# marella/ctransformers

Measured on NVIDIA H100. Metric: decode tokens/s Llama-2-7B Q4_K_M b=1, higher is better.
Workload: dtype int8 (q4_K/q6_K weights x q8_K activations, mma.sync u8 x s8 -> exact int32), fp32 combine in the reference's order

## Files before the change

ctransformers_b200/csrc/engine.cu:

```cuda
#include "engine.cuh"

#include <algorithm>
#include <chrono>
#include <cstdio>
#include <cstring>
#include <stdexcept>

#include "attention.cuh"
#include "matvec.cuh"
#include "prefill.cuh"
#include "repack.cuh"
#include "sample_gpu.cuh"
#include "stream.cuh"
#include "tables.hpp"
#include "tp_nccl.hpp"

namespace ctb {

#define CTB_CUDA(expr)                                                                                         \
  do {                                                                                                         \
    cudaError_t e__ = (expr);                                                                                  \
    if (e__ != cudaSuccess)                                                                                    \
      throw std::runtime_error(std::string("CUDA error: ") + cudaGetErrorString(e__) + " at " + __FILE__ + ":" + \
                               std::to_string(__LINE__) + " (" #expr ")" + watchdog_note());                   \
// ... 775 lines not shown
  if (launches) *launches = (long)sel.size();
  stream_ = user; launches_per_step_ = keep;
  cudaStreamDestroy(cap);
  cudaEvent_t e0, e1;
  CTB_CUDA(cudaEventCreate(&e0)); CTB_CUDA(cudaEventCreate(&e1));
  for (int i = 0; i < 3; i++) CTB_CUDA(cudaGraphLaunch(ex, stream_));
  CTB_CUDA(cudaEventRecord(e0, stream_));
  for (int i = 0; i < reps; i++) CTB_CUDA(cudaGraphLaunch(ex, stream_));
  CTB_CUDA(cudaEventRecord(e1, stream_));
  CTB_CUDA(cudaStreamSynchronize(stream_));
  float ms = 0;
  cudaEventElapsedTime(&ms, e0, e1);
  cudaEventDestroy(e0); cudaEventDestroy(e1); cudaGraphExecDestroy(ex);
  return (double)ms / reps;
}

long Engine::trace_step(int token, int n_past, unsigned long long* out, long cap_words) {
  DeviceGuard dev_guard(device_);
  if (tp_.world > 1) throw std::runtime_error("not available in tensor-parallel mode (every rank must run the same launches)");
  spec_pending_ = false; spec_deferred_ = false; spec_pos_ = -1; spec_streak_ = 0;
  const int n = n_body_ + 1;
  for (int i = 0; i < n; i++)
    if (ops_[i].ph.kind == PH_MATVEC && !ops_[i].stream) return 0;
  const long need = 2L * n + 8L * n * step_grid_;
  if (need > cap_words) return -need;
  unsigned long long* buf = nullptr;
  CTB_CUDA(cudaMalloc(&buf, (size_t)n * step_grid_ * 64));
  CTB_CUDA(cudaMemset(buf, 0, (size_t)n * step_grid_ * 64));
  StepLaunch L;
  L.grid = step_grid_; L.n_slots = step_slots_; L.smem = step_smem_; L.gen = !attn_fast_hd(hp_.head_dim());
  if (h_state_cap_ < 1) { h_state_cap_ = 512; CTB_CUDA(cudaMallocHost(&h_state_, (size_t)h_state_cap_ * 16)); }
  for (int rep = 0; rep < 3; rep++) {
    h_state_[0] = token; h_state_[1] = n_past; h_state_[2] = 0; h_state_[3] = n_past + 1;
    CTB_CUDA(cudaMemcpyAsync(d_state_, h_state_, 16, cudaMemcpyHostToDevice, stream_));
    CTB_CUDA(launch_step(L, stream_, d_prog_, d_bounds_, n, d_sync_, false, buf));
    CTB_CUDA(cudaStreamSynchronize(stream_));
  }
  for (int i = 0; i < n; i++) { out[2 * i] = (unsigned long long)ops_[i].ph.kind; out[2 * i + 1] = (unsigned long long)ops_[i].mvk; }
  const cudaError_t e = cudaMemcpy(out + 2 * n, buf, (size_t)n * step_grid_ * 64, cudaMemcpyDeviceToHost);
  cudaFree(buf);
  CTB_CUDA(e);
  return n;
}

void Engine::destroy_graphs() {
  if (graph_full_) cudaGraphExecDestroy(graph_full_);
  if (graph_nolog_) cudaGraphExecDestroy(graph_nolog_);
  if (graph_greedy_) cudaGraphExecDestroy(graph_greedy_);
  graph_full_ = graph_nolog_ = graph_greedy_ = nullptr;
}

void Engine::build_graphs() {
  destroy_graphs();
  if (!d_tokens_out_) {
    tokens_out_cap_ = std::max(hp_.n_ctx, 4096);
    CTB_CUDA(cudaMalloc(&d_tokens_out_, (size_t)tokens_out_cap_ * 4));
    CTB_CUDA(cudaMallocHost(&h_tokens_out_, (size_t)tokens_out_cap_ * 4));
  }
  cudaStream_t user = stream_;
  cudaStream_t cap;
  CTB_CUDA(cudaStreamCreateWithFlags(&cap, cudaStreamNonBlocking));
  stream_ = cap;
// ... 309 lines not shown
```

ctransformers_b200/csrc/matvec.cuh:

```cuda
#pragma once
#include "device_types.cuh"
#include "attention.cuh"

namespace ctb {

#ifndef CTB_THREADS
#define CTB_THREADS 512
#endif
constexpr int MV_THREADS = CTB_THREADS;
constexpr int MV_WARPS = MV_THREADS / 32;
constexpr int MV_ROWS = 4;
constexpr int MV_MAX_SEG = 3;

enum : int { NORM_NONE = 0, NORM_RMS = 1, NORM_LAYER = 2 };
enum : int { EPI_STORE = 0, EPI_ADD = 1, EPI_GELU = 2, EPI_ADD2 = 3, EPI_SILU = 4 };

#ifndef ST_WATCHDOG_NS
#define ST_WATCHDOG_NS 4000000000ull
#endif
#ifndef XC_WATCHDOG_NS
#define XC_WATCHDOG_NS 30000000000ull
#endif
enum WaitCode : int {
  W_GRID_BARRIER = 1, W_FOLD_FLAG, W_FREE_WEIGHT_SLOT, W_WEIGHT_ITEM, W_FREE_K_SLOT, W_FREE_V_SLOT, W_K_ITEM, W_V_ITEM, W_XCHG,
// ... 73 lines not shown
  return a;
}

__device__ __forceinline__ int q8k_word_offset(int b, int s, int l) { return ((b * 2 + (s >> 2)) * 8 + l) * 16 + (s & 3) * 4; }


template <bool CG = false>
__device__ __forceinline__ void load16(const float* p, int valid, float (&v)[16]) {
  if (valid >= 16) {
    float4 a, b, c, d;
    if (CG) { a = __ldcg((const float4*)p); b = __ldcg((const float4*)p + 1); c = __ldcg((const float4*)p + 2); d = __ldcg((const float4*)p + 3); }
    else { a = __ldg((const float4*)p); b = __ldg((const float4*)p + 1); c = __ldg((const float4*)p + 2); d = __ldg((const float4*)p + 3); }
    v[0] = a.x; v[1] = a.y; v[2] = a.z; v[3] = a.w; v[4] = b.x; v[5] = b.y; v[6] = b.z; v[7] = b.w;
    v[8] = c.x; v[9] = c.y; v[10] = c.z; v[11] = c.w; v[12] = d.x; v[13] = d.y; v[14] = d.z; v[15] = d.w;
  } else {
#pragma unroll
    for (int e = 0; e < 16; e++) v[e] = e < valid ? (CG ? __ldcg(p + e) : __ldg(p + e)) : 0.f;
  }
}

template <int NT, int BAR>
__device__ __forceinline__ double block_sum_f64(double s, double* red ) {
  s = warp_sum(s);
  bar_sync<BAR, NT>();
  if ((threadIdx.x & 31) == 0) red[threadIdx.x >> 5] = s;
  bar_sync<BAR, NT>();
  double t = 0.0;
#pragma unroll
  for (int w = 0; w < NT / 32; w++) t += red[w];
  return t;
}
template <int NT, int BAR>
__device__ __forceinline__ void block_sum2_max_f64(double& s, double& a, double& g, double* red) {
  constexpr int NW = NT / 32;
#pragma unroll
  for (int o = 16; o > 0; o >>= 1) {
    s += __shfl_xor_sync(0xffffffffu, s, o);
    a += __shfl_xor_sync(0xffffffffu, a, o);
    g = fmax(g, __shfl_xor_sync(0xffffffffu, g, o));
  }
  bar_sync<BAR, NT>();
  if ((threadIdx.x & 31) == 0) { red[threadIdx.x >> 5] = s; red[NW + (threadIdx.x >> 5)] = a; red[2 * NW + (threadIdx.x >> 5)] = g; }
  bar_sync<BAR, NT>();
  s = 0.0;
  a = 0.0;
#pragma unroll
  for (int w = 0; w < NW; w++) { s += red[w]; a += red[NW + w]; g = fmax(g, red[2 * NW + w]); }
}

__device__ __forceinline__ uint32_t pack4(const int* q) {
  return (uint32_t)(q[0] & 0xff) | ((uint32_t)(q[1] & 0xff) << 8) | ((uint32_t)(q[2] & 0xff) << 16) | ((uint32_t)(q[3] & 0xff) << 24);
}

__device__ __forceinline__ void load16_ll(const uint2* p, unsigned epoch, float (&u)[16]) {
  uint4 q[8];
  bounded_wait([&] {
    bool ok = true;
#pragma unroll
    for (int j = 0; j < 8; j++) {
      asm volatile("ld.volatile.global.v4.u32 {%0,%1,%2,%3}, [%4];" : "=r"(q[j].x), "=r"(q[j].y), "=r"(q[j].z), "=r"(q[j].w) : "l"(p + 2 * j) : "memory");
    }
#pragma unroll
    for (int j = 0; j < 8; j++) ok &= q[j].y == epoch && q[j].w == epoch;
    return ok;
// ... 52 lines not shown
  double seq = 0.0;
  for (int base = 0; base < K; base += 512) {
    float v[16];
    load16x<XC>(xs, base + lane * 16, K - base - lane * 16, v, epoch);
    for (int l = 0; l < 32; l++)
#pragma unroll
      for (int i = 0; i < 16; i++) {
        float t = __shfl_sync(0xffffffffu, v[i], l);
        if (kind == NORM_TERM_DEV) t = __fsub_rn(t, mean);
        if (base + l * 16 + i < K) seq += kind == NORM_TERM_X ? (double)t : (double)__fmul_rn(t, t);
      }
  }
  return seq;
}

template <int NT, int BAR, bool XC>
__device__ __forceinline__ float norm_stat(double s, double a, double g, bool a_is_s, int kind, float mean, const MVParams& xs, double* red,
                                           unsigned epoch) {
  const int K = xs.K;
  if (a_is_s) a = s = block_sum_f64<NT, BAR>(s, red);
  else block_sum2_max_f64<NT, BAR>(s, a, g, red);
  if (!isfinite(s) || (!a_is_s && __dmul_ru(a, g) < 0x1p52)) return (float)(s / (double)K);
  const double e = __dmul_ru(a, (double)K * 0x1.0000001p-52);
  const float lo = (float)(__dsub_rd(s, e) / (double)K), hi = (float)(__dadd_ru(s, e) / (double)K);
  if (lo == hi) return lo;
  const double seq = threadIdx.x < 32 ? seq_sum_warp0<XC>(xs.x, xs.x2, xs.x_mode, xs.x_parts, xs.x_stride, K, kind, mean, epoch) : 0.0;
  bar_sync<BAR, NT>();
  if (threadIdx.x == 0) red[0] = seq;
  bar_sync<BAR, NT>();
  return (float)(red[0] / (double)K);
}

template <int NT, int BAR, bool XC = false>
__device__ __forceinline__ void stage_activation(const MVParams& xs, const NormPre& np, int act, uint8_t* smem, double* red, bool write_norm, unsigned epoch = 0) {
  const float* nw = xs.norm_w;
  const float* nb_ = xs.norm_b;
  float* norm_out = xs.norm_out;
  const int norm_mode = xs.norm_mode, K = xs.K;
  const float eps = xs.eps;
  const int t = threadIdx.x, lane = t & 31;
  const int passes = (K + NT * 16 - 1) / (NT * 16);
  float mean = 0.f, scale = 1.f;
  float v0[16];
  load16x<XC>(xs, t * 16, K - t * 16, v0, epoch);
  if (norm_mode == NORM_RMS) {
    double ss = 0.0;
    for (int ps = 0; ps < passes; ps++) {
      const int base = (ps * NT + t) * 16;
      if ((base & ~511) >= K) continue;
      float v[16];
      if (ps == 0) {
#pragma unroll
        for (int e = 0; e < 16; e++) v[e] = v0[e];
      } else load16x<XC>(xs, base, K - base, v, epoch);
#pragma unroll
      for (int e = 0; e < 16; e++) ss += (double)__fmul_rn(v[e], v[e]);
    }
    const float m = norm_stat<NT, BAR, XC>(ss, ss, 0.0, true, NORM_TERM_SQ, 0.f, xs, red, epoch);
    scale = __fdiv_rn(1.0f, __fsqrt_rn(__fadd_rn(m, eps)));
  } else if (norm_mode == NORM_LAYER) {
    double s1 = 0.0, a1 = 0.0;
    unsigned emin = 255;
    for (int ps = 0; ps < passes; ps++) {
      const int base = (ps * NT + t) * 16;
      if ((base & ~511) >= K) continue;
      float v[16];
      load16x<XC>(xs, base, K - base, v, epoch);
#pragma unroll
      for (int e = 0; e < 16; e++) {
        s1 += (double)v[e];
        a1 += (double)fabsf(v[e]);
        emin = min_exp(emin, v[e]);
      }
    }
    mean = norm_stat<NT, BAR, XC>(s1, a1, lsb_inv(emin), false, NORM_TERM_X, 0.f, xs, red, epoch);
    double s2 = 0.0;
    for (int ps = 0; ps < passes; ps++) {
      const int base = (ps * NT + t) * 16;
      if ((base & ~511) >= K) continue;
      float v[16];
      load16x<XC>(xs, base, K - base, v, epoch);
#pragma unroll
      for (int e = 0; e < 16; e++) { const float d = (base + e < K) ? __fsub_rn(v[e], mean) : 0.f; s2 += (double)__fmul_rn(d, d); }
    }
    const float var = norm_stat<NT, BAR, XC>(s2, s2, 0.0, true, NORM_TERM_DEV, mean, xs, red, epoch);
    scale = __fdiv_rn(1.0f, __fsqrt_rn(__fadd_rn(var, eps)));
  }
  int8_t* qs = (int8_t*)smem;
  const size_t off = ((size_t)K + 15) & ~(size_t)15;
  float* dd = (float*)(smem + off);
  int16_t* bs = (int16_t*)(smem + off + q8k_d_bytes(K));
  for (int ps = 0; ps < passes; ps++) {
    const int base = (ps * NT + t) * 16;
    const int valid = K - base;
    if ((base & ~511) >= K) continue;
    float v[16];
    if (ps == 0) {
#pragma unroll
      for (int e = 0; e < 16; e++) v[e] = v0[e];
    } else load16x<XC>(xs, base, valid, v, epoch);
    if (XC && write_norm && xs.x_mode == 2 && xs.sum_out && valid > 0) {
#pragma unroll
      for (int e = 0; e < 16; e++) if (e < valid) xs.sum_out[base + e] = v[e];
    }
    if (norm_mode != NORM_NONE) {
      float w[16], bb[16];
      if (ps == 0) {
#pragma unroll
        for (int e = 0; e < 16; e++) { w[e] = np.w0[e]; bb[e] = np.bias0[e]; }
      } else {
// ... 5 lines not shown
        float y = v[e];
        if (norm_mode == NORM_LAYER) y = __fsub_rn(y, mean);
        y = __fmul_rn(y, scale);
        if (nw) y = __fmul_rn(y, w[e]);
        if (nb_) y = __fadd_rn(y, bb[e]);
        v[e] = y;
      }
    }
    if (write_norm && norm_out && valid > 0) {
#pragma unroll
      for (int e = 0; e < 16; e++) if (e < valid) norm_out[base + e] = v[e];
    }
    if (act == ACT_Q8_K) {
      float amax = 0.f, mx = 0.f;
#pragma unroll
      for (int e = 0; e < 16; e++) { const float ax = fabsf(v[e]); if (ax > amax) { amax = ax; mx = v[e]; } }
      float gmax = amax;
#pragma unroll
      for (int o = 8; o > 0; o >>= 1) gmax = fmaxf(gmax, __shfl_xor_sync(0xffffffffu, gmax, o));
      const unsigned who = __ballot_sync(0xffffffffu, amax == gmax);
      const int hbase = lane & 16, hl = lane & 15;
      const unsigned mine = (who >> hbase) & 0xffffu;
      const float maxv = __shfl_sync(0xffffffffu, mx, hbase + __ffs(mine) - 1);
      if (valid > 0) {
        const int b = base >> 8;
        int q[16];
        int sum = 0;
        if (gmax == 0.f) {
#pragma unroll
          for (int e = 0; e < 16; e++) q[e] = 0;
          if (hl == 0) dd[b] = 0.f;
        } else {
          const float iscale = __fdiv_rn(-128.f, maxv);
#pragma unroll
          for (int e = 0; e < 16; e++) {
            const float val = __fmaf_rn(iscale, v[e], 12582912.f);
            q[e] = min(127, (__float_as_int(val) & 0x007fffff) - 0x00400000);
            sum += q[e];
          }
          if (hl == 0) dd[b] = __fdiv_rn(1.f, iscale);
        }
        bs[b * 16 + hl] = (int16_t)sum;
#pragma unroll
        for (int j = 0; j < 4; j++) {
          const int wi = hl * 4 + j;
          *(uint32_t*)(qs + q8k_word_offset(b, wi >> 3, wi & 7)) = pack4(q + 4 * j);
        }
      }
    } else if (act == ACT_Q8_0) {
      float amax = 0.f;
#pragma unroll
      for (int e = 0; e < 16; e++) amax = fmaxf(amax, fabsf(v[e]));
      amax = fmaxf(amax, __shfl_xor_sync(0xffffffffu, amax, 1));
      if (valid > 0) {
        const float d = __fdiv_rn(amax, 127.f);
        const float id = amax != 0.f ? __fdiv_rn(127.f, amax) : 0.f;
        int q[16];
#pragma unroll
        for (int e = 0; e < 16; e++) q[e] = __float2int_rn(__fmul_rn(v[e], id));
        *(uint4*)(qs + base) = make_uint4(pack4(q), pack4(q + 4), pack4(q + 8), pack4(q + 12));
        if ((lane & 1) == 0) dd[base >> 5] = h2f(f2h(d));
      }
    } else if (act == ACT_Q8_1) {
      float amax = 0.f;
#pragma unroll
      for (int e = 0; e < 16; e++) amax = fmaxf(amax, fabsf(v[e]));
      amax = fmaxf(amax, __shfl_xor_sync(0xffffffffu, amax, 1));
      const float d = __fdiv_rn(amax, 127.f);
      const float id = amax != 0.f ? __fdiv_rn(127.f, amax) : 0.f;
      int q[16];
      int sum = 0;
#pragma unroll
      for (int e = 0; e < 16; e++) { q[e] = __float2int_rn(__fmul_rn(v[e], id)); sum += q[e]; }
      sum += __shfl_xor_sync(0xffffffffu, sum, 1);
      if (valid > 0) {
        *(uint4*)(qs + base) = make_uint4(pack4(q), pack4(q + 4), pack4(q + 8), pack4(q + 12));
        if ((lane & 1) == 0) *(float2*)(dd + (base >> 4)) = make_float2(d, __fmul_rn(d, (float)sum));
      }
    } else if (act == ACT_F16) {
      uint16_t* h = (uint16_t*)smem;
#pragma unroll
      for (int e = 0; e < 16; e++) if (e < valid) h[base + e] = f2h(v[e]);
    } else {
      float* f = (float*)smem;
#pragma unroll
      for (int e = 0; e < 16; e++) if (e < valid) f[base + e] = v[e];
    }
  }
  bar_sync<BAR, NT>();
}

__device__ __forceinline__ float group_hsum8(float v) {
  v = v + __shfl_xor_sync(0xffffffffu, v, 4);
  v = v + __shfl_xor_sync(0xffffffffu, v, 2);
  v = v + __shfl_xor_sync(0xffffffffu, v, 1);
  return v;
}

__device__ __forceinline__ float dot_q40(const DevMat& w, int row, const ActView& a, int l) {
  const int nb = w.nb;
  const uint8_t* qrow = w.qs + (size_t)row * nb * 16 + (l & 3) * 4;
  const uint16_t* drow = w.d + (size_t)row * nb;
  const int shift = (l >> 2) * 4;
  float acc = 0.f;
#pragma unroll 8
  for (int b = 0; b < nb; b++) {
    const uint32_t q = (uint32_t)__ldg((const int*)(qrow + (size_t)b * 16));
    const float dw = h2f(__ldg(drow + b));
    const int aw = *(const int*)(a.qs + b * 32 + l * 4);
    const float yd = a.d[b];
    const uint32_t nib = (q >> shift) & 0x0f0f0f0fu;
    const uint32_t bx = ((nib | 0x80808080u) - 0x08080808u) ^ 0x80808080u;
// ... 98 lines not shown
  const int np = w.K & ~31;
  float s = 0.f;
  for (int i = lane; i < np; i += 32) s = __fmaf_rn(__ldg(wr + i), xa[i], s);
  float sumf = warp_reduce_f32x8(s);
  for (int i = np; i < w.K; i++) sumf = __fmaf_rn(__ldg(wr + i), xa[i], sumf);
  return sumf;
}

__device__ __forceinline__ float table_f16(const uint16_t* tab, float x) { return h2f(__ldg(tab + f2h(x))); }

__device__ __forceinline__ float epilogue(int epi, float v, const float* res, const float* res2, const MVParams& p) {
  if (epi == EPI_ADD) return __fadd_rn(v, __ldcg(res));
  if (epi == EPI_ADD2) return __fadd_rn(__fadd_rn(v, __ldcg(res)), __ldcg(res2));
  if (epi == EPI_GELU) return table_f16(p.gelu_tab, v);
  if (epi == EPI_SILU) return table_f16(p.silu_tab, v);
  return v;
}
__device__ __forceinline__ void store_epilogue(const MVSeg& sg, const MVParams& p, int row, float v) { sg.out[row] = epilogue(sg.epi, v, sg.res + row, sg.res2 + row, p); }

__host__ __device__ inline int rows_per_unit(int type) { return (type == GT_F16 || type == GT_F32) ? 1 : MV_ROWS; }

static __global__ void __launch_bounds__(MV_THREADS, 1) k_matvec(const __grid_constant__ MVParams p) {
  extern __shared__ __align__(16) uint8_t smem[];
  __shared__ double red[3 * MV_WARPS];
  const int warp = threadIdx.x >> 5, lane = threadIdx.x & 31;
  pdl_trigger();
  NormPre np;
  preload_norm(np, p);
  pdl_wait();
  stage_activation<MV_THREADS, 0>(p, np, p.act, smem, red, blockIdx.x == 0);
  const ActView a = act_view(p.act, p.K, smem);
  const int gw = blockIdx.x * MV_WARPS + warp, nw = gridDim.x * MV_WARPS;
  int first = gw;
  for (int s = 0; s < p.nseg; s++) {
    const MVSeg& sg = p.seg[s];
    const int type = sg.w.type;
    const int rpu = rows_per_unit(type);
    const int units = (sg.w.M + rpu - 1) / rpu;
    int un = first;
    for (; un < units; un += nw) {
      if (rpu == 1) {
        const float v = type == GT_F16 ? dot_f16_row(sg.w, un, smem, lane) : dot_f32_row(sg.w, un, smem, lane);
        if (lane == 0) store_epilogue(sg, p, un, v);
      } else {
        const int row = un * MV_ROWS + (lane >> 3);
        const float v = dot_legacy(sg.w, min(row, sg.w.M - 1), a, lane & 7);
        if ((lane & 7) == 0 && row < sg.w.M) store_epilogue(sg, p, row, v);
// ... 26 lines not shown
```

ctransformers_b200/csrc/ops_abi.cu:

```cuda
#include <cmath>
#include <cstdio>
#include <cstring>
#include <functional>
#include <memory>
#include <stdexcept>
#include <string>
#include <vector>

#include "../../include/ctransformers_b200.h"
#include "attention.cuh"
#include "matvec.cuh"
#include "prefill.cuh"
#include "repack.cuh"
#include "stream.cuh"
#include "tables.hpp"

using namespace ctb;

namespace {

#define OPS_CUDA(expr)                                                                                     \
  do {                                                                                                     \
    cudaError_t e__ = (expr);                                                                              \
    if (e__ != cudaSuccess) throw std::runtime_error(std::string("CUDA error: ") + cudaGetErrorString(e__) + " (" #expr ")"); \
// ... 95 lines not shown
  OPS_CUDA(cudaGetLastError());
  OPS_CUDA(cudaDeviceSynchronize());
}

void run_matvec(MVParams& p) {
  p.silu_tab = tables().silu;
  p.gelu_tab = tables().gelu;
  if (step_supports(p)) {
    run_phases({matvec_phase(p)});
    return;
  }
  static bool attr = false;
  if (!attr) {
    OPS_CUDA(matvec_set_smem_limit(MV_SMEM_LIMIT));
    attr = true;
  }
  const MVLaunch L = matvec_launch_shape(p, sm_count());
  OPS_CUDA(launch_matvec_kernel(L, 0, p));
  OPS_CUDA(cudaGetLastError());
}

__global__ void __launch_bounds__(MV_THREADS) k_stage_dump(const __grid_constant__ MVParams q, int act, uint8_t* dump) {
  extern __shared__ __align__(16) uint8_t smem[];
  __shared__ double red[3 * MV_WARPS];
  NormPre np;
  preload_norm(np, q);
  stage_activation<MV_THREADS, 0>(q, np, act, smem, red, true);
  const size_t n = act_smem_bytes(act, q.K);
  for (size_t i = threadIdx.x; i < n; i += MV_THREADS) dump[i] = smem[i];
}

__global__ void __launch_bounds__(MV_THREADS) k_gate_dump(const __grid_constant__ MVParams q, float* out) {
  extern __shared__ __align__(16) uint8_t smem[];
  __shared__ double red[3 * MV_WARPS];
  NormPre np;
  preload_norm(np, q);
  stage_activation<MV_THREADS, 0>(q, np, ACT_F32, smem, red, false);
  const float* f = (const float*)smem;
  for (int i = threadIdx.x; i < q.K; i += MV_THREADS) out[i] = f[i];
}

__global__ void k_rope_dump(float* x, const float2* rope, int pos, int hd, int neox) {
  float* row = x + (size_t)blockIdx.x * hd;
  int i0, i1;
  float o0, o1;
  rope_head_pair(row, threadIdx.x, hd, neox, rope[(size_t)pos * (hd / 2) + threadIdx.x], i0, i1, o0, o1);
  row[i0] = o0; row[i1] = o1;
}

int guarded(const char* what, const std::function<void()>& fn) {
  try {
    int ndev = 0;
    if (cudaGetDeviceCount(&ndev) != cudaSuccess || ndev == 0) throw std::runtime_error("no CUDA device available (no CPU fallback)");
    fn();
    return 0;
  } catch (const std::exception& e) {
    fprintf(stderr, "ctransformers-b200: %s failed: %s\n", what, e.what());
// ... 421 lines not shown
```

ctransformers_b200/csrc/prefill.cuh:

```cuda
#pragma once
#include "stream.cuh"

namespace ctb {

constexpr int PB_T = 32;
constexpr int PB_TG = PB_T / 8;
constexpr int PB_TEAMS = 2;
constexpr int PB_W = PB_TEAMS * 4;
constexpr int PB_NT = PB_W * 32;
constexpr int PB_THREADS = PB_NT + 32;
constexpr int PB_BAR = 1;
constexpr int PB_XCH = 12 * 16 * PB_T * 4;

enum : int { PP_EMBED = 0, PP_QUANT = 1, PP_GEMM = 2, PP_KV = 3, PP_ATTN = 4 };

__host__ __device__ inline size_t pb_qbuf_bytes(int K) { return (size_t)(K / 256) * (8192 + 512 + 128); }

struct alignas(16) PPhase {
  int kind;
  MVParams mv;
  int x_ld, x2_ld;
  int out_ld[MV_MAX_SEG], res_ld[MV_MAX_SEG], res2_ld[MV_MAX_SEG];
  uint8_t* qbuf;
  AttnParams at;
// ... 311 lines not shown
  for (int c = 0; c < hd; c++) {
    const float o = attn_vp(p.vc + v_chan(kvh, c, p.n_ctx, hd), s.p16, a, -1, 0);
    if (lane == 0) orow[c] = o;
  }
  __syncwarp();
}

template <bool GEN>
__device__ __forceinline__ void pb_attn_phase(const PPhase& ph, int n_tok, uint8_t* work) {
  const int warp = threadIdx.x >> 5;
  const int n_tasks = n_tok * ph.at.n_head;
  uint8_t* wsm = work + (size_t)warp * pb_attn_warp_bytes(ph.at.n_ctx, ph.at.hd);
  for (int task = blockIdx.x * PB_W + warp; task < n_tasks; task += (int)gridDim.x * PB_W) {
    const int tok = task / ph.at.n_head;
    pb_attn_warp_task<GEN>(ph.at, ph.state + tok * 4, tok, task % ph.at.n_head, wsm);
  }
}
static __device__ __noinline__ void pb_attn_phase_gen(const PPhase& ph, int n_tok, uint8_t* work) { pb_attn_phase<true>(ph, n_tok, work); }

static __global__ void __launch_bounds__(PB_THREADS, 1) k_pstep(const __grid_constant__ PStepArgs args) {
  extern __shared__ __align__(16) uint8_t smem[];
  __shared__ __align__(8) uint64_t full_bar[ST_MAX_SLOTS];
  __shared__ __align__(8) uint64_t empty_bar[ST_MAX_SLOTS];
  __shared__ double red[3 * PB_W];
  __shared__ __align__(16) PPhase ph;
  const int warp = threadIdx.x >> 5;
  uint8_t* ring = smem;
  uint8_t* work = smem + (size_t)args.n_slots * ST_SLOT;
  ring_init(full_bar, empty_bar, args.n_slots, 4);
  if (warp == PB_W) {
    pb_producer(args, ring, full_bar, empty_bar);
    return;
  }
  const unsigned G = gridDim.x;
  uint32_t seq = 0;
#pragma unroll 1
  for (int ip = 0; ip < args.n_phases; ip++) {
    bar_sync<PB_BAR, PB_NT>();
    if (threadIdx.x == 0 && ip > 0) { __threadfence(); atomicAdd(args.sync, 1u); }
    {
      const uint4* src = (const uint4*)(args.prog + ip);
      uint4* dst = (uint4*)&ph;
      for (int i = threadIdx.x - 32; i >= 0 && i < (int)(sizeof(PPhase) / 16); i += PB_NT - 32) dst[i] = __ldg(src + i);
    }
    bar_sync<PB_BAR, PB_NT>();
    if (threadIdx.x == 0 && ip > 0) {
      const unsigned target = (unsigned)ip * G;
// ... 68 lines not shown
```

ctransformers_b200/csrc/stream.cuh:

```cuda
#pragma once
#include "matvec.cuh"

namespace ctb {

#ifndef CTB_ST_WARPS
#define CTB_ST_WARPS 10
#endif
constexpr int ST_W = CTB_ST_WARPS;
constexpr int ST_NT = ST_W * 32;
constexpr int ST_THREADS = ST_NT + 32;
constexpr int ST_SLOT = 9216;
#ifndef CTB_ST_DEPTH
#define CTB_ST_DEPTH 2
#endif
constexpr int ST_MAX_DEPTH = CTB_ST_DEPTH;
constexpr int ST_MAX_SLOTS = ST_W * ST_MAX_DEPTH;
constexpr int ST_MAXT = 16;
constexpr int ST_ROWS = 16;
constexpr int ST_BAR = 1;
constexpr int ST_STATE = 6;

#ifndef CTB_CHUNK_Q4
#define CTB_CHUNK_Q4 4
#endif
// ... 98 lines not shown
__device__ __forceinline__ uint64_t l2_policy_evict_first() {
  uint64_t p;
  asm volatile("createpolicy.fractional.L2::evict_first.b64 %0, 1.0;" : "=l"(p));
  return p;
}
__device__ __forceinline__ void mma_u8s8(int (&d)[4], uint32_t a0, uint32_t a1, uint32_t a2, uint32_t a3, uint32_t b0, uint32_t b1, int c0, int c1) {
  asm("mma.sync.aligned.m16n8k32.row.col.s32.u8.s8.s32 {%0,%1,%2,%3}, {%4,%5,%6,%7}, {%8,%9}, {%10,%11,%12,%13};"
      : "=r"(d[0]), "=r"(d[1]), "=r"(d[2]), "=r"(d[3])
      : "r"(a0), "r"(a1), "r"(a2), "r"(a3), "r"(b0), "r"(b1), "r"(c0), "r"(c1), "r"(c0), "r"(c1));
}

struct StAct {
  const int8_t* qs;
  const float* d;
  const uint32_t* pairs;
  const int* cneg;
  const int8_t* zero;
  const struct XchgParams* xc;
  unsigned epoch;
};
__host__ __device__ inline size_t st_off_pairs(int K) { return ((((size_t)K + 15) & ~(size_t)15) + q8k_d_bytes(K) + (size_t)(K / 16) * 2 + 15) & ~(size_t)15; }
__host__ __device__ inline size_t st_act_bytes(int K, bool q6) { return st_off_pairs(K) + (size_t)(K / 256) * 16 + (q6 ? (size_t)K : 0) + 256 + 16; }

template <int NT, int BAR>
__device__ __forceinline__ StAct st_act_extras(uint8_t* smem, int K, bool q6) {
  const ActView a = act_view(ACT_Q8_K, K, smem);
  StAct s;
  s.qs = a.qs; s.d = a.d;
  uint32_t* pairs = (uint32_t*)(smem + st_off_pairs(K));
  int* cneg = (int*)(smem + st_off_pairs(K) + (size_t)(K / 256) * 16);
  s.pairs = pairs; s.cneg = cneg;
  const int nb = K >> 8;
  int* zero = (int*)(smem + st_off_pairs(K) + (size_t)nb * 16 + (q6 ? (size_t)K : 0));
  s.zero = (const int8_t*)zero;
  if (threadIdx.x < 64) zero[threadIdx.x] = 0;
  for (int i = threadIdx.x; i < nb * 4; i += NT) {
    const int16_t* b4 = a.bs + (i >> 2) * 16 + 4 * (i & 3);
    const int p0 = (int)b4[0] + (int)b4[1], p1 = (int)b4[2] + (int)b4[3];
    pairs[i] = (uint32_t)(p0 & 0xffff) | ((uint32_t)p1 << 16);
  }
  if (q6) {
    for (int i = threadIdx.x; i < nb * 64; i += NT) {
      const int b = i >> 6, grp = (i >> 3) & 7, l = i & 7;
      const int w = *(const int*)(a.qs + q8k_word_offset(b, grp, l));
      cneg[((b * 4 + (l >> 1)) * 8 + grp) * 2 + (l & 1)] = -32 * __dp4a(0x01010101, w, 0);
    }
  }
  bar_sync<BAR, NT>();
  return s;
}

__device__ __forceinline__ void unpack_k4(uint32_t s0, uint32_t s1, uint32_t s2, uint32_t& sc03, uint32_t& sc47, uint32_t& m03, uint32_t& m47) {
  sc03 = s0 & 0x3f3f3f3fu;
  m03 = s1 & 0x3f3f3f3fu;
  sc47 = (s2 & 0x0f0f0f0fu) | (((s0 >> 6) & 0x03030303u) << 4);
  m47 = ((s2 >> 4) & 0x0f0f0f0fu) | (((s1 >> 6) & 0x03030303u) << 4);
}
__device__ __forceinline__ int pack16(int lo, int hi) { return (int)__byte_perm((uint32_t)lo, (uint32_t)hi, 0x5410); }
__device__ __forceinline__ int scale_fold8(int d0, int d1, int d2, int d3, int d4, int d5, int d6, int d7, uint32_t s03, uint32_t s47) {
  int s = __dp2a_lo(pack16(d0, d1), (int)s03, 0);
  s = __dp2a_hi(pack16(d2, d3), (int)s03, s);
  s = __dp2a_lo(pack16(d4, d5), (int)s47, s);
  s = __dp2a_hi(pack16(d6, d7), (int)s47, s);
  return s;
}

struct Terms { float p[4]; float pm[2]; float dd[2]; float ddm[2]; };

__device__ __forceinline__ void load_b_operands(const StAct& a, int b, int g, int t, uint32_t (&bA)[8], uint32_t (&bB)[8]) {
  const int8_t* word = a.qs + b * 256 + g * 16;
  const int8_t* pa = (g == t) ? word : a.zero;
// ... 264 lines not shown
  int world, rank, index, n;
  int role;
  uint2* ll[XC_MAX_WORLD];
};
struct PickParams { const float* logits; int* state; int* out_tokens; int n; };
struct alignas(16) Phase {
  int kind;
  int q6;
  MVParams mv;
  AttnParams at;
  EmbedParams em;
  PickParams pk;
  XchgParams xc;
};

struct StepArgs {
  const Phase* prog;
  int n_phases;
  int n_slots;
  unsigned* sync;
  const int* bounds;
  unsigned long long* trace;
};

__device__ __forceinline__ unsigned ld_relaxed_u32(const unsigned* p) {
  unsigned v;
  asm volatile("ld.relaxed.gpu.global.u32 %0, [%1];" : "=r"(v) : "l"(p) : "memory");
  return v;
}
__device__ __forceinline__ unsigned ld_acquire_u32(const unsigned* p) {
  unsigned v;
  asm volatile("ld.acquire.gpu.global.u32 %0, [%1];" : "=r"(v) : "l"(p) : "memory");
  return v;
}

struct TileInfo { int seg, til, nch, type; };
__device__ __forceinline__ TileInfo tile_info(const TileSpace& ts, const MVParams& p, int tile, int nb, bool valid) {
  TileInfo ti;
  ti.seg = 0; ti.til = 0; ti.nch = 0; ti.type = GT_Q4_K;
  if (valid) {
    int tl = tile;
    ti.seg = ts.locate(tl);
    ti.til = tl;
    ti.type = ti.seg == 0 ? p.seg[0].w.type : (ti.seg == 1 ? p.seg[1].w.type : p.seg[2].w.type);
    ti.nch = st_chunks(ti.type, nb);
  }
// ... 162 lines not shown
            const uint32_t n = seq + (uint32_t)rank;
            const RingPos rp = st_ring(n, S);
            const StItem it = st_item(p, ti.seg, ti.type, ti.til, kc, nb);
            mbar_wait(&empty_bar[rp.slot], rp.parity ^ 1u, W_FREE_WEIGHT_SLOT, (int)n);
            mbar_expect_tx(&full_bar[rp.slot], it.bytes);
            bulk_g2s_hint(ring + (size_t)rp.slot * ST_SLOT, it.src, it.bytes, &full_bar[rp.slot], weight_pol);
          }
          __syncwarp();
        }
        __syncwarp();
        seq += (uint32_t)__popc(mask);
      }
    }
  }
}

template <bool XC>
__device__ __forceinline__ void st_matvec_phase(const Phase& ph, const NormPre& np, uint8_t* ring, uint8_t* act_smem, double* red, uint64_t* full_bar, uint64_t* empty_bar,
                                                float (*mailbox)[ST_STATE * 32], int* flags, uint32_t S, uint32_t& seq, const int* tb, unsigned long long* tr,
                                                unsigned xc_base) {
  const MVParams& p = ph.mv;
  const int warp = threadIdx.x >> 5, lane = threadIdx.x & 31;
  const unsigned epoch = XC ? xc_base + (unsigned)ph.xc.index + 1u : 0u;
  stage_activation<ST_NT, ST_BAR, XC>(p, np, ACT_Q8_K, act_smem, red, blockIdx.x == 0, epoch);
  StAct a = st_act_extras<ST_NT, ST_BAR>(act_smem, p.K, ph.q6 != 0);
  a.xc = XC && ph.xc.role == 2 ? &ph.xc : nullptr;
  a.epoch = epoch;
  if (tr && threadIdx.x == 0) tr[1] = globaltimer_ns();
  bool first_item = tr != nullptr && threadIdx.x == 0;
  TileSpace ts;
  ts.init(p);
  const int nb = p.K >> 8;
  const int T0 = tb[0], T1 = tb[1];
#pragma unroll 1
  for (int w0 = T0; w0 < T1; w0 += ST_MAXT) {
    if (w0 != T0) {
      bar_sync<ST_BAR, ST_NT>();
      if (threadIdx.x < ST_MAXT) flags[threadIdx.x] = 0;
      bar_sync<ST_BAR, ST_NT>();
    }
    const int ntw = min(ST_MAXT, T1 - w0);
    const TileInfo ti = tile_info(ts, p, w0 + lane, nb, lane < ntw);
#pragma unroll 1
    for (int kc = 0;; kc++) {
      const unsigned mask = __ballot_sync(0xffffffffu, kc < ti.nch);
      if (!mask) break;
      const int cnt = __popc(mask);
#pragma unroll 1
// ... 30 lines not shown
  if (threadIdx.x == 0) {
    pk.state[4] = idx;
    advance_state(pk.state, pk.out_tokens, idx);
  }
}

__device__ __forceinline__ void grid_rearm(unsigned* sync, bool set_xc = false, unsigned xc = 0) {
  if (threadIdx.x == 0) {
    __threadfence();
    if (atomicAdd(sync + 1, 1u) == gridDim.x - 1) {
      sync[0] = 0u;
      sync[1] = 0u;
      if (set_xc) sync[2] = xc;
      __threadfence();
    }
  }
}

template <bool XC, bool GEN>
static __global__ void __launch_bounds__(ST_THREADS, 1) k_step(const __grid_constant__ StepArgs args) {
  extern __shared__ __align__(16) uint8_t smem[];
  __shared__ __align__(8) uint64_t full_bar[ST_MAX_SLOTS];
  __shared__ __align__(8) uint64_t empty_bar[ST_MAX_SLOTS];
  __shared__ double red[3 * ST_W];
  __shared__ __align__(16) float mailbox[ST_MAXT][ST_STATE * 32];
  __shared__ int flags[ST_MAXT];
  __shared__ float pick_v[ST_W];
  __shared__ int pick_i[ST_W];
  __shared__ __align__(16) Phase ph_s[2];
  __shared__ int tb_s[2][2];
  const int warp = threadIdx.x >> 5;
  uint8_t* ring = smem;
  uint8_t* act_smem = smem + (size_t)args.n_slots * ST_SLOT;
  ring_init(full_bar, empty_bar, args.n_slots, 1);
  pdl_trigger();
  pdl_wait();
  if (warp == ST_W) {
    st_producer<XC, GEN>(args, ring, full_bar, empty_bar);
    return;
  }
  const unsigned G = gridDim.x;
  uint32_t seq = 0;
  const unsigned xc_base = XC ? ld_relaxed_u32(args.sync + 2) : 0u;
  unsigned xc_done = 0;
  auto fetch_phase = [&](int ip) {
    if (ip >= args.n_phases) return;
    const uint4* src = (const uint4*)(args.prog + ip);
    const uint32_t dst = st_smem(&ph_s[ip & 1]);
    const int i = (int)threadIdx.x - 32;
    if (i >= 0 && i < (int)(sizeof(Phase) / 16)) asm volatile("cp.async.ca.shared.global [%0], [%1], 16;" ::"r"(dst + i * 16), "l"(src + i) : "memory");
    if (i >= 64 && i < 66)
      asm volatile("cp.async.ca.shared.global [%0], [%1], 4;" ::"r"(st_smem(&tb_s[ip & 1][i - 64])), "l"(args.bounds + (size_t)ip * (gridDim.x + 1) + blockIdx.x + (i - 64)) : "memory");
    asm volatile("cp.async.commit_group;" ::: "memory");
  };
  fetch_phase(0);
#pragma unroll 1
  for (int ip = 0; ip < args.n_phases; ip++) {
    bar_sync<ST_BAR, ST_NT>();
    unsigned long long* const tr = args.trace ? args.trace + ((size_t)ip * G + blockIdx.x) * 8 : nullptr;
    if (tr && threadIdx.x == 0) tr[4] = globaltimer_ns();
    if (threadIdx.x == 0 && ip > 0) {
      const unsigned target = (unsigned)ip * G;
      asm volatile("red.release.gpu.global.add.u32 [%0], 1;" ::"l"(args.sync) : "memory");
      if (tr) tr[5] = globaltimer_ns();
      bounded_wait([&] { return ld_relaxed_u32(args.sync) >= target; }, W_GRID_BARRIER, ip);
      if (tr) { tr[6] = globaltimer_ns(); tr[7] = tr[6]; }
    } else {
      asm volatile("cp.async.wait_all;" ::: "memory");
      if (threadIdx.x >= 32 && threadIdx.x < 32 + ST_MAXT) flags[threadIdx.x - 32] = 0;
    }
    bar_sync<ST_BAR, ST_NT>();
    const Phase& ph = ph_s[ip & 1];
    fetch_phase(ip + 1);
    NormPre np;
    if (ph.kind == PH_MATVEC) preload_norm(np, ph.mv);
    if (tr && threadIdx.x == 0) tr[0] = globaltimer_ns();
    if (XC && ph.kind == PH_MATVEC && ph.xc.role == 1) xc_done++;
    if (ph.kind == PH_MATVEC) {
      st_matvec_phase<XC>(ph, np, ring, act_smem, red, full_bar, empty_bar, mailbox, flags, (uint32_t)(args.n_slots / ST_W), seq, &tb_s[ip & 1][0], tr, xc_base);
    } else if (ph.kind == PH_ATTN) {
      if (GEN) seq = st_attn_phase_gen(ph, act_smem, ring, full_bar, empty_bar, args.n_slots, seq, pick_v, red);
      else st_attn_phase<false>(ph, act_smem, ring, full_bar, empty_bar, args.n_slots, seq, pick_v, red);
    } else if (ph.kind == PH_EMBED) {
      if (blockIdx.x == 0) embed_row(ph.em, ph.em.tokens[0], ph.em.out, threadIdx.x, ST_NT);
    } else if (ph.kind == PH_PICK) {
      if (blockIdx.x == 0) st_pick_phase(ph.pk, pick_v, pick_i);
    }
    if (tr) {
      bar_sync<ST_BAR, ST_NT>();
      if (threadIdx.x == 0) tr[3] = globaltimer_ns();
    }
  }
  bar_sync<ST_BAR, ST_NT>();
  grid_rearm(args.sync, XC, xc_base + xc_done);
}

struct StepLaunch { int grid; int n_slots; size_t smem; bool gen = false;  };

// ... 62 lines not shown
```

Before: 357.6.

## Fuse q8_K pair sums and q6 cneg into activation staging, trim barriers

After: 360.4 (median of 6 runs). About the same (+0.8%).

```diff
diff --git a/ctransformers_b200/csrc/engine.cu b/ctransformers_b200/csrc/engine.cu
--- a/ctransformers_b200/csrc/engine.cu
+++ b/ctransformers_b200/csrc/engine.cu
@@ -821,11 +821,12 @@
   const int n = n_body_ + 1;
   for (int i = 0; i < n; i++)
     if (ops_[i].ph.kind == PH_MATVEC && !ops_[i].stream) return 0;
-  const long need = 2L * n + 8L * n * step_grid_;
+  const long need = 2L * n + (long)ST_TRACE_WORDS * n * step_grid_;
   if (need > cap_words) return -need;
+  const size_t bytes = (size_t)n * step_grid_ * ST_TRACE_WORDS * 8;
   unsigned long long* buf = nullptr;
-  CTB_CUDA(cudaMalloc(&buf, (size_t)n * step_grid_ * 64));
-  CTB_CUDA(cudaMemset(buf, 0, (size_t)n * step_grid_ * 64));
+  CTB_CUDA(cudaMalloc(&buf, bytes));
+  CTB_CUDA(cudaMemset(buf, 0, bytes));
   StepLaunch L;
   L.grid = step_grid_; L.n_slots = step_slots_; L.smem = step_smem_; L.gen = !attn_fast_hd(hp_.head_dim());
   if (h_state_cap_ < 1) { h_state_cap_ = 512; CTB_CUDA(cudaMallocHost(&h_state_, (size_t)h_state_cap_ * 16)); }
@@ -836,7 +837,7 @@
     CTB_CUDA(cudaStreamSynchronize(stream_));
   }
   for (int i = 0; i < n; i++) { out[2 * i] = (unsigned long long)ops_[i].ph.kind; out[2 * i + 1] = (unsigned long long)ops_[i].mvk; }
-  const cudaError_t e = cudaMemcpy(out + 2 * n, buf, (size_t)n * step_grid_ * 64, cudaMemcpyDeviceToHost);
+  const cudaError_t e = cudaMemcpy(out + 2 * n, buf, bytes, cudaMemcpyDeviceToHost);
   cudaFree(buf);
   CTB_CUDA(e);
   return n;
diff --git a/ctransformers_b200/csrc/matvec.cuh b/ctransformers_b200/csrc/matvec.cuh
--- a/ctransformers_b200/csrc/matvec.cuh
+++ b/ctransformers_b200/csrc/matvec.cuh
@@ -119,7 +119,6 @@
 template <int NT, int BAR>
 __device__ __forceinline__ double block_sum_f64(double s, double* red ) {
   s = warp_sum(s);
-  bar_sync<BAR, NT>();
   if ((threadIdx.x & 31) == 0) red[threadIdx.x >> 5] = s;
   bar_sync<BAR, NT>();
   double t = 0.0;
@@ -136,7 +135,6 @@
     a += __shfl_xor_sync(0xffffffffu, a, o);
     g = fmax(g, __shfl_xor_sync(0xffffffffu, g, o));
   }
-  bar_sync<BAR, NT>();
   if ((threadIdx.x & 31) == 0) { red[threadIdx.x >> 5] = s; red[NW + (threadIdx.x >> 5)] = a; red[2 * NW + (threadIdx.x >> 5)] = g; }
   bar_sync<BAR, NT>();
   s = 0.0;
@@ -235,7 +233,15 @@
   else block_sum2_max_f64<NT, BAR>(s, a, g, red);
   if (!isfinite(s) || (!a_is_s && __dmul_ru(a, g) < 0x1p52)) return (float)(s / (double)K);
   const double e = __dmul_ru(a, (double)K * 0x1.0000001p-52);
-  const float lo = (float)(__dsub_rd(s, e) / (double)K), hi = (float)(__dadd_ru(s, e) / (double)K);
+  float lo, hi;
+  if ((K & (K - 1)) == 0) {
+    const double rk = __longlong_as_double((long long)(1023 + 1 - __ffs(K)) << 52);
+    lo = (float)__dmul_rn(__dsub_rd(s, e), rk);
+    hi = (float)__dmul_rn(__dadd_ru(s, e), rk);
+  } else {
+    lo = (float)(__dsub_rd(s, e) / (double)K);
+    hi = (float)(__dadd_ru(s, e) / (double)K);
+  }
   if (lo == hi) return lo;
   const double seq = threadIdx.x < 32 ? seq_sum_warp0<XC>(xs.x, xs.x2, xs.x_mode, xs.x_parts, xs.x_stride, K, kind, mean, epoch) : 0.0;
   bar_sync<BAR, NT>();
@@ -244,8 +250,16 @@
   return (float)(red[0] / (double)K);
 }
 
-template <int NT, int BAR, bool XC = false>
-__device__ __forceinline__ void stage_activation(const MVParams& xs, const NormPre& np, int act, uint8_t* smem, double* red, bool write_norm, unsigned epoch = 0) {
+struct Q8KExtras { uint32_t* pairs; int* cneg; };
+
+template <int NT> constexpr int RED_STAT1 = 3 * NT / 32;
+template <int NT> constexpr int RED_DOUBLES = 4 * NT / 32;
+
+enum : int { TR_STAGE_LOADED = 8, TR_STAGE_STAT = 9, TR_STAGE_QUANT = 10, TR_STAGE_DONE = 11 };
+
+template <int NT, int BAR, bool XC = false, bool EX = false>
+__device__ __forceinline__ void stage_activation(const MVParams& xs, const NormPre& np, int act, uint8_t* smem, double* red, bool write_norm, unsigned epoch = 0,
+                                                 Q8KExtras ex = {}, unsigned long long* tr = nullptr) {
   const float* nw = xs.norm_w;
   const float* nb_ = xs.norm_b;
   float* norm_out = xs.norm_out;
@@ -269,6 +283,7 @@
 #pragma unroll
       for (int e = 0; e < 16; e++) ss += (double)__fmul_rn(v[e], v[e]);
     }
+    if (tr && t == 0) tr[TR_STAGE_LOADED] = globaltimer_ns();
     const float m = norm_stat<NT, BAR, XC>(ss, ss, 0.0, true, NORM_TERM_SQ, 0.f, xs, red, epoch);
     scale = __fdiv_rn(1.0f, __fsqrt_rn(__fadd_rn(m, eps)));
   } else if (norm_mode == NORM_LAYER) {
@@ -286,6 +301,7 @@
         emin = min_exp(emin, v[e]);
       }
     }
+    if (tr && t == 0) tr[TR_STAGE_LOADED] = globaltimer_ns();
     mean = norm_stat<NT, BAR, XC>(s1, a1, lsb_inv(emin), false, NORM_TERM_X, 0.f, xs, red, epoch);
     double s2 = 0.0;
     for (int ps = 0; ps < passes; ps++) {
@@ -296,9 +312,12 @@
 #pragma unroll
       for (int e = 0; e < 16; e++) { const float d = (base + e < K) ? __fsub_rn(v[e], mean) : 0.f; s2 += (double)__fmul_rn(d, d); }
     }
-    const float var = norm_stat<NT, BAR, XC>(s2, s2, 0.0, true, NORM_TERM_DEV, mean, xs, red, epoch);
+    const float var = norm_stat<NT, BAR, XC>(s2, s2, 0.0, true, NORM_TERM_DEV, mean, xs, red + RED_STAT1<NT>, epoch);
     scale = __fdiv_rn(1.0f, __fsqrt_rn(__fadd_rn(var, eps)));
-  }
+  } else if (tr && t == 0) {
+    tr[TR_STAGE_LOADED] = globaltimer_ns();
+  }
+  if (tr && t == 0) tr[TR_STAGE_STAT] = globaltimer_ns();
   int8_t* qs = (int8_t*)smem;
   const size_t off = ((size_t)K + 15) & ~(size_t)15;
   float* dd = (float*)(smem + off);
@@ -350,10 +369,10 @@
       const int hbase = lane & 16, hl = lane & 15;
       const unsigned mine = (who >> hbase) & 0xffffu;
       const float maxv = __shfl_sync(0xffffffffu, mx, hbase + __ffs(mine) - 1);
+      const int b = base >> 8;
+      int sum = 0;
       if (valid > 0) {
-        const int b = base >> 8;
         int q[16];
-        int sum = 0;
         if (gmax == 0.f) {
 #pragma unroll
           for (int e = 0; e < 16; e++) q[e] = 0;
@@ -374,6 +393,19 @@
           const int wi = hl * 4 + j;
           *(uint32_t*)(qs + q8k_word_offset(b, wi >> 3, wi & 7)) = pack4(q + 4 * j);
         }
+        if (EX && ex.cneg) {
+          int c[4];
+#pragma unroll
+          for (int j = 0; j < 4; j++) c[j] = -32 * (q[4 * j] + q[4 * j + 1] + q[4 * j + 2] + q[4 * j + 3]);
+          int* cn = ex.cneg + ((b * 4 + (hl & 1) * 2) * 8 + (hl >> 1)) * 2;
+          *(int2*)cn = make_int2(c[0], c[1]);
+          *(int2*)(cn + 16) = make_int2(c[2], c[3]);
+        }
+      }
+      if (EX) {
+        const int s2 = sum + __shfl_xor_sync(0xffffffffu, sum, 1);
+        const int s4 = __shfl_xor_sync(0xffffffffu, s2, 2);
+        if (valid > 0 && (hl & 3) == 0) ex.pairs[b * 4 + (hl >> 2)] = (uint32_t)(s2 & 0xffff) | ((uint32_t)s4 << 16);
       }
     } else if (act == ACT_Q8_0) {
       float amax = 0.f;
@@ -415,7 +447,9 @@
       for (int e = 0; e < 16; e++) if (e < valid) f[base + e] = v[e];
     }
   }
+  if (tr && t == 0) tr[TR_STAGE_QUANT] = globaltimer_ns();
   bar_sync<BAR, NT>();
+  if (tr && t == 0) tr[TR_STAGE_DONE] = globaltimer_ns();
 }
 
 __device__ __forceinline__ float group_hsum8(float v) {
@@ -560,7 +594,7 @@
 
 static __global__ void __launch_bounds__(MV_THREADS, 1) k_matvec(const __grid_constant__ MVParams p) {
   extern __shared__ __align__(16) uint8_t smem[];
-  __shared__ double red[3 * MV_WARPS];
+  __shared__ double red[RED_DOUBLES<MV_THREADS>];
   const int warp = threadIdx.x >> 5, lane = threadIdx.x & 31;
   pdl_trigger();
   NormPre np;
diff --git a/ctransformers_b200/csrc/ops_abi.cu b/ctransformers_b200/csrc/ops_abi.cu
--- a/ctransformers_b200/csrc/ops_abi.cu
+++ b/ctransformers_b200/csrc/ops_abi.cu
@@ -141,7 +141,7 @@
 
 __global__ void __launch_bounds__(MV_THREADS) k_stage_dump(const __grid_constant__ MVParams q, int act, uint8_t* dump) {
   extern __shared__ __align__(16) uint8_t smem[];
-  __shared__ double red[3 * MV_WARPS];
+  __shared__ double red[RED_DOUBLES<MV_THREADS>];
   NormPre np;
   preload_norm(np, q);
   stage_activation<MV_THREADS, 0>(q, np, act, smem, red, true);
@@ -151,7 +151,7 @@
 
 __global__ void __launch_bounds__(MV_THREADS) k_gate_dump(const __grid_constant__ MVParams q, float* out) {
   extern __shared__ __align__(16) uint8_t smem[];
-  __shared__ double red[3 * MV_WARPS];
+  __shared__ double red[RED_DOUBLES<MV_THREADS>];
   NormPre np;
   preload_norm(np, q);
   stage_activation<MV_THREADS, 0>(q, np, ACT_F32, smem, red, false);
diff --git a/ctransformers_b200/csrc/prefill.cuh b/ctransformers_b200/csrc/prefill.cuh
--- a/ctransformers_b200/csrc/prefill.cuh
+++ b/ctransformers_b200/csrc/prefill.cuh
@@ -357,7 +357,7 @@
   extern __shared__ __align__(16) uint8_t smem[];
   __shared__ __align__(8) uint64_t full_bar[ST_MAX_SLOTS];
   __shared__ __align__(8) uint64_t empty_bar[ST_MAX_SLOTS];
-  __shared__ double red[3 * PB_W];
+  __shared__ double red[RED_DOUBLES<PB_NT>];
   __shared__ __align__(16) PPhase ph;
   const int warp = threadIdx.x >> 5;
   uint8_t* ring = smem;
diff --git a/ctransformers_b200/csrc/stream.cuh b/ctransformers_b200/csrc/stream.cuh
--- a/ctransformers_b200/csrc/stream.cuh
+++ b/ctransformers_b200/csrc/stream.cuh
@@ -144,31 +144,17 @@
 __host__ __device__ inline size_t st_off_pairs(int K) { return ((((size_t)K + 15) & ~(size_t)15) + q8k_d_bytes(K) + (size_t)(K / 16) * 2 + 15) & ~(size_t)15; }
 __host__ __device__ inline size_t st_act_bytes(int K, bool q6) { return st_off_pairs(K) + (size_t)(K / 256) * 16 + (q6 ? (size_t)K : 0) + 256 + 16; }
 
-template <int NT, int BAR>
-__device__ __forceinline__ StAct st_act_extras(uint8_t* smem, int K, bool q6) {
+__device__ __forceinline__ StAct st_act_layout(uint8_t* smem, int K, bool q6, Q8KExtras& ex) {
   const ActView a = act_view(ACT_Q8_K, K, smem);
   StAct s;
   s.qs = a.qs; s.d = a.d;
-  uint32_t* pairs = (uint32_t*)(smem + st_off_pairs(K));
-  int* cneg = (int*)(smem + st_off_pairs(K) + (size_t)(K / 256) * 16);
-  s.pairs = pairs; s.cneg = cneg;
   const int nb = K >> 8;
+  ex.pairs = (uint32_t*)(smem + st_off_pairs(K));
+  ex.cneg = q6 ? (int*)(smem + st_off_pairs(K) + (size_t)nb * 16) : nullptr;
+  s.pairs = ex.pairs; s.cneg = ex.cneg;
   int* zero = (int*)(smem + st_off_pairs(K) + (size_t)nb * 16 + (q6 ? (size_t)K : 0));
   s.zero = (const int8_t*)zero;
   if (threadIdx.x < 64) zero[threadIdx.x] = 0;
-  for (int i = threadIdx.x; i < nb * 4; i += NT) {
-    const int16_t* b4 = a.bs + (i >> 2) * 16 + 4 * (i & 3);
-    const int p0 = (int)b4[0] + (int)b4[1], p1 = (int)b4[2] + (int)b4[3];
-    pairs[i] = (uint32_t)(p0 & 0xffff) | ((uint32_t)p1 << 16);
-  }
-  if (q6) {
-    for (int i = threadIdx.x; i < nb * 64; i += NT) {
-      const int b = i >> 6, grp = (i >> 3) & 7, l = i & 7;
-      const int w = *(const int*)(a.qs + q8k_word_offset(b, grp, l));
-      cneg[((b * 4 + (l >> 1)) * 8 + grp) * 2 + (l & 1)] = -32 * __dp4a(0x01010101, w, 0);
-    }
-  }
-  bar_sync<BAR, NT>();
   return s;
 }
 
@@ -479,6 +465,7 @@
   const int* bounds;
   unsigned long long* trace;
 };
+constexpr int ST_TRACE_WORDS = 12;
 
 __device__ __forceinline__ unsigned ld_relaxed_u32(const unsigned* p) {
   unsigned v;
@@ -687,8 +674,9 @@
   const MVParams& p = ph.mv;
   const int warp = threadIdx.x >> 5, lane = threadIdx.x & 31;
   const unsigned epoch = XC ? xc_base + (unsigned)ph.xc.index + 1u : 0u;
-  stage_activation<ST_NT, ST_BAR, XC>(p, np, ACT_Q8_K, act_smem, red, blockIdx.x == 0, epoch);
-  StAct a = st_act_extras<ST_NT, ST_BAR>(act_smem, p.K, ph.q6 != 0);
+  Q8KExtras ex;
+  StAct a = st_act_layout(act_smem, p.K, ph.q6 != 0, ex);
+  stage_activation<ST_NT, ST_BAR, XC, true>(p, np, ACT_Q8_K, act_smem, red, blockIdx.x == 0, epoch, ex, tr);
   a.xc = XC && ph.xc.role == 2 ? &ph.xc : nullptr;
   a.epoch = epoch;
   if (tr && threadIdx.x == 0) tr[1] = globaltimer_ns();
@@ -765,7 +753,7 @@
   extern __shared__ __align__(16) uint8_t smem[];
   __shared__ __align__(8) uint64_t full_bar[ST_MAX_SLOTS];
   __shared__ __align__(8) uint64_t empty_bar[ST_MAX_SLOTS];
-  __shared__ double red[3 * ST_W];
+  __shared__ double red[RED_DOUBLES<ST_NT>];
   __shared__ __align__(16) float mailbox[ST_MAXT][ST_STATE * 32];
   __shared__ int flags[ST_MAXT];
   __shared__ float pick_v[ST_W];
@@ -799,8 +787,10 @@
   fetch_phase(0);
 #pragma unroll 1
   for (int ip = 0; ip < args.n_phases; ip++) {
+    NormPre np;
+    if (args.prog[ip].kind == PH_MATVEC) preload_norm(np, args.prog[ip].mv);
     bar_sync<ST_BAR, ST_NT>();
-    unsigned long long* const tr = args.trace ? args.trace + ((size_t)ip * G + blockIdx.x) * 8 : nullptr;
+    unsigned long long* const tr = args.trace ? args.trace + ((size_t)ip * G + blockIdx.x) * ST_TRACE_WORDS : nullptr;
     if (tr && threadIdx.x == 0) tr[4] = globaltimer_ns();
     if (threadIdx.x == 0 && ip > 0) {
       const unsigned target = (unsigned)ip * G;
@@ -815,8 +805,6 @@
     bar_sync<ST_BAR, ST_NT>();
     const Phase& ph = ph_s[ip & 1];
     fetch_phase(ip + 1);
-    NormPre np;
-    if (ph.kind == PH_MATVEC) preload_norm(np, ph.mv);
     if (tr && threadIdx.x == 0) tr[0] = globaltimer_ns();
     if (XC && ph.kind == PH_MATVEC && ph.xc.role == 1) xc_done++;
     if (ph.kind == PH_MATVEC) {
```
